# fy-vision/DiGA

Measured on AMD Instinct MI355X. Metric: 768x768 19-class crops/sec (DiGA warm-up step), higher is better.
Workload: dtype f32; 1 GPU; configs[1]: ResNet-101 DeepLabV2 DiGA warm-up (student + EMA teacher, KL distill), synthetic GTA5-shape 768x768, batch 8 per GPU; global_batch=8, parallelism=dp1

## Files before the change

### diga_amd/csrc/conv.hip

```cpp
#include <stdlib.h>
#include <string.h>

#include <algorithm>
#include <atomic>

#include "common.h"

namespace diga {

using f32x16 = __attribute__((ext_vector_type(16))) float;
using f32x4nt = __attribute__((ext_vector_type(4))) float;

__device__ __forceinline__ void store4_stream(float* p, float x, float y, float z, float w) {
#if defined(DIGA_PROBE_NOSTORE)
    if (x == 1.2345e38f) *p = y + z + w;
#elif defined(DIGA_PROBE_PLAINSTORE)
    *reinterpret_cast<float4*>(p) = make_float4(x, y, z, w);
#else
    __builtin_nontemporal_store((f32x4nt){x, y, z, w}, reinterpret_cast<f32x4nt*>(p));
#endif
}

constexpr int kBK = 32;

// ... 1051 lines not shown
#pragma unroll
        for (int j = 0; j < NT; ++j)
#pragma unroll
            for (int e = 0; e < 4; ++e)
                stage[((wm & 1) * 64 + i * 16 + (lane >> 4) * 4 + e) * LDS_LD + wn * 32 * TN + j * 16 + (lane & 15)] = acc[i][j][e];
    __syncthreads();
    drain_stage<2, TN, EPI>(stage, a, m0 + h * 128, n0, t, tile_m * 2 + h, m0 + h * 128 < a.M);
}

#if defined(DIGA_PROBE_STAMP)
__device__ unsigned long long g_probe_stamps[8192 * 6];
#define DIGA_STAMP(slot_)                                                                                                  \
    do {                                                                                                                   \
        if (wv == 0 && lane == 0 && blockIdx.x < 8192) {                                                                   \
            __builtin_amdgcn_sched_barrier(0);                                                                             \
            g_probe_stamps[blockIdx.x * 6 + (slot_)] = __builtin_amdgcn_s_memrealtime();                                   \
            __builtin_amdgcn_sched_barrier(0);                                                                             \
        }                                                                                                                  \
    } while (0)
#else
#define DIGA_STAMP(slot_) do { } while (0)
#endif

#ifndef DIGA_FWD_DMA_MINW
#define DIGA_FWD_DMA_MINW 3
#endif
template <bool EPI = false>
__global__ __launch_bounds__(768, DIGA_FWD_DMA_MINW) void conv_fwd_dma_kernel(ConvArgs a) {
    constexpr int BM = 256, BN = 128;
    constexpr int A_BYTES = BM * 128, B_BYTES = BN * 128, STAGE = A_BYTES + B_BYTES;
    extern __shared__ __align__(16) unsigned char smem_b[];
    const int lane = threadIdx.x & 63, wv = threadIdx.x >> 6;
    const bool loader = wv >= 8;
    DIGA_STAMP(0);
    const int wg = xcd_remap(blockIdx.x, gridDim.x);
    const int tile_n = wg % a.tiles_n, tile_m = wg / a.tiles_n;
    const int m0 = tile_m * BM, n0 = tile_n * BN;
    const int RS = a.R * a.S;
    const int cchunks = a.Cin / 32;
    const uint64_t live = RS <= 64 ? live_taps(a, m0, BM) : ~0ull;
    const int ntaps = RS <= 64 ? __builtin_popcountll(live) : RS;
    const int ksteps = ntaps * cchunks;

    if (loader) {
        const int lw = wv - 8;
        const unsigned char* in_b = reinterpret_cast<const unsigned char*>(a.in);
        const int lrow = lane >> 3;
        int pixbase[8], yx0[8];
        bool mok[8];
        const int HoWo = a.Ho * a.Wo;
#pragma unroll
        for (int j = 0; j < 8; ++j) {
            const int m = m0 + lw * 64 + 8 * j + lrow;
            mok[j] = m < a.M;
            const int mm = mok[j] ? m : a.M - 1;
            const int img = mm / HoWo, rem = mm - img * HoWo;
            const int ho = rem / a.Wo, wo = rem - ho * a.Wo;
            pixbase[j] = img * a.Hi * a.Wi;
            yx0[j] = ((ho * a.sy + a.oy0) << 16) | ((wo * a.sx + a.ox0) & 0xffff);
        }
        const int64_t rowb = (int64_t)a.in_ld * 4;
        const unsigned char* pa[8];
        const unsigned char* pb[4];
#pragma unroll
        for (int c = 0; c < 4; ++c) {
            const int r = lw * 32 + 8 * c + lrow, co = n0 + r;
            const int chunk = (lane & 7) ^ ((r >> 1) & 7);
            const float* wbase = a.wb_tiles > 0 ? a.wgt + (int64_t)(tile_m / a.wb_tiles) * a.wb_stride : a.wgt;
            pb[c] = co < a.Cout ? reinterpret_cast<const unsigned char*>(wbase) + (int64_t)co * RS * a.Cin * 4 + chunk * 16 : nullptr;
        }
        uint64_t todo = live;
        int l_tap = 0, l_cc = 0;
        auto next_tap = [&]() {
            if (RS <= 64) {
                l_tap = __builtin_ctzll(todo);
                todo &= todo - 1;
            } else {
                ++l_tap;
            }
        };
        auto set_tap = [&](int tap) {
            const int r = tap / a.S, q = tap - r * a.S;
            const int dy = r * a.ody, dx = q * a.odx;
#pragma unroll
            for (int j = 0; j < 8; ++j) {
                const int iy = (yx0[j] >> 16) + dy, ix = (int)(short)(yx0[j] & 0xffff) + dx;
                int cy, cx;
                const bool ok = map_tap(a, iy, ix, cy, cx) && mok[j];
                const int chunk = (lane & 7) ^ (((8 * j + lrow) >> 1) & 7);
                pa[j] = ok ? in_b + (int64_t)(pixbase[j] + cy * a.Wi + cx) * rowb + chunk * 16 : nullptr;
            }
        };
        int issued = 0;
        auto issue = [&](int buf) {
            unsigned char* stage = smem_b + buf * STAGE;
#pragma unroll
            for (int j = 0; j < 8; ++j) {
                const unsigned char* src = pa[j] != nullptr ? pa[j] + l_cc * 128 : g_zero16;
                __builtin_amdgcn_global_load_lds((const __attribute__((address_space(1))) void*)src,
                                                 (__attribute__((address_space(3))) void*)(stage + (lw * 64 + 8 * j) * 128), 16, 0, 0);
            }
            const int64_t boff = ((int64_t)l_tap * a.Cin + l_cc * 32) * 4;
#pragma unroll
            for (int c = 0; c < 4; ++c) {
                const unsigned char* src = pb[c] != nullptr ? pb[c] + boff : g_zero16;
                __builtin_amdgcn_global_load_lds((const __attribute__((address_space(1))) void*)src,
                                                 (__attribute__((address_space(3))) void*)(stage + A_BYTES + (lw * 32 + 8 * c) * 128), 16, 0, 0);
            }
            ++issued;
            if (++l_cc == cchunks) {
                l_cc = 0;
                if (issued < ksteps) {
                    next_tap();
                    set_tap(l_tap);
                }
            }
        };
        auto wait_next = [&](bool newest_in_flight) {
            if (newest_in_flight) asm volatile("s_waitcnt vmcnt(12)" ::: "memory");
            else asm volatile("s_waitcnt vmcnt(0)" ::: "memory");
            __builtin_amdgcn_s_barrier();
        };
        if (RS <= 64) next_tap();
        set_tap(l_tap);
        issue(0);
        if (ksteps > 1) issue(1);
        wait_next(ksteps > 1);
        int nx = 2;
        for (int ks = 0; ks < ksteps; ++ks) {
            const bool ahead = ks + 2 < ksteps;
            if (ahead) issue(nx);
            wait_next(ahead);
            nx = nx == 2 ? 0 : nx + 1;
        }
        return;
    }

    const int wm = wv >> 1, wn = wv & 1;
    f32x16 acc[2][2];
#pragma unroll
    for (int i = 0; i < 2; ++i)
#pragma unroll
        for (int j = 0; j < 2; ++j)
// ... 737 lines not shown
#pragma unroll
            for (int j = 0; j < NT; ++j) acc[i][j] = __builtin_amdgcn_mfma_f32_16x16x32_bf16(ah, bh[j], acc[i][j], 0, 0, 0);
        }
        asm volatile("s_waitcnt lgkmcnt(0)" ::: "memory");
        __builtin_amdgcn_s_barrier();
        cur = cur == 2 ? 0 : cur + 1;
    }

    float* out = a.slab + (int64_t)split * a.Cout * RS * a.Cin;
#pragma unroll
    for (int j = 0; j < NT; ++j) {
        const int c = c0 + wn * 64 + j * 16 + (lane & 15);
#pragma unroll
        for (int i = 0; i < MT; ++i) {
#pragma unroll
            for (int e = 0; e < 4; ++e) {
                const int kk = k0 + wm * 128 + i * 16 + (lane >> 4) * 4 + e;
                if (kk < a.Cout && c < a.Cin) out[((int64_t)kk * RS + tap) * a.Cin + c] = acc[i][j][e];
            }
        }
    }
}

__global__ __launch_bounds__(768, 3) void conv_wgrad_dma_kernel(WgradArgs a) {
    constexpr int BM = 256, BN = 128;
    constexpr int A_ROW = BM * 4, B_ROW = BN * 4;
    constexpr int A_BYTES = kBK * A_ROW, B_BYTES = kBK * B_ROW, STAGE = A_BYTES + B_BYTES;
    extern __shared__ __align__(16) unsigned char smem_b[];
    const int lane = threadIdx.x & 63, wv = threadIdx.x >> 6;
    const bool loader = wv >= 8;
    const int RS = a.R * a.S;
    int wg = xcd_remap(blockIdx.x, gridDim.x);
    const int tile_n = wg % a.tiles_n;
    wg /= a.tiles_n;
    const int tile_m = wg % a.tiles_m;
    wg /= a.tiles_m;
    const int tap = wg % RS;
    const int split = wg / RS;
    const int k0 = tile_m * BM, c0 = tile_n * BN;
    const int p_begin = split * a.steps_per_split * kBK;
    int p_end = p_begin + a.steps_per_split * kBK;
    if (p_end > a.M) p_end = a.M;
    const int ksteps = p_end > p_begin ? (p_end - p_begin + kBK - 1) / kBK : 0;

    if (loader) {
        const int lw = wv - 8;
        const unsigned char* dyb = reinterpret_cast<const unsigned char*>(a.dy) + ((int64_t)k0 + tap * a.dy_tap_stride) * 4;
        const unsigned char* xb = reinterpret_cast<const unsigned char*>(a.x) + ((int64_t)c0 + tap * a.x_tap_stride) * 4;
        const int64_t dy_rowb = (int64_t)a.dy_ld * 4, x_rowb = (int64_t)a.x_ld * 4;
        const int* tab = a.ptab != nullptr ? a.ptab + (int64_t)tap * a.M_pad : nullptr;
        const int b_half = lane >> 5;
        const int b_src = (((lane & 31) ^ (b_half << 3)) << 4);
        int bidx[4];
        auto load_idx = [&](int ks) {
#pragma unroll
            for (int j = 0; j < 4; ++j) {
                const int p = p_begin + ks * kBK + 8 * lw + 2 * j + b_half;
                bidx[j] = p < p_end ? (tab != nullptr ? tab[p] : p) : -1;
            }
        };
        auto issue = [&](int ks, int stg) {
            unsigned char* stage = smem_b + stg * STAGE;
#pragma unroll
            for (int j = 0; j < 8; ++j) {
                const int row = 8 * lw + j;
                const int p = min(p_begin + ks * kBK + row, a.M - 1);
                const unsigned char* src = dyb + p * dy_rowb + ((lane ^ ((j & 1) << 3)) << 4);
                __builtin_amdgcn_global_load_lds((const __attribute__((address_space(1))) void*)src,
                                                 (__attribute__((address_space(3))) void*)(stage + row * A_ROW), 16, 0, 0);
            }
#pragma unroll
            for (int j = 0; j < 4; ++j) {
                const unsigned char* src = bidx[j] >= 0 ? xb + bidx[j] * x_rowb + b_src : g_zero16;
                __builtin_amdgcn_global_load_lds((const __attribute__((address_space(1))) void*)src,
                                                 (__attribute__((address_space(3))) void*)(stage + A_BYTES + (8 * lw + 2 * j) * B_ROW), 16, 0, 0);
            }
        };
        auto wait_next = [&](bool newest_in_flight) {
            if (newest_in_flight) asm volatile("s_waitcnt vmcnt(12)" ::: "memory");
            else asm volatile("s_waitcnt vmcnt(0)" ::: "memory");
            __builtin_amdgcn_s_barrier();
        };
        if (ksteps > 0) {
            load_idx(0);
            issue(0, 0);
            if (ksteps > 1) {
                load_idx(1);
                issue(1, 1);
            }
        }
        wait_next(ksteps > 1);
        int nx = 2;
        for (int ks = 0; ks < ksteps; ++ks) {
            const bool ahead = ks + 2 < ksteps;
            if (ahead) {
                load_idx(ks + 2);
                issue(ks + 2, nx);
            }
            wait_next(ahead);
            nx = nx == 2 ? 0 : nx + 1;
        }
        return;
    }
// ... 131 lines not shown
    DIGA_REQUIRE(!e->mask_bits || e->mask_bits_ld * 8 >= a.Cout, DIGA_EINVAL, "%s: bad mask_bits", who);
    DIGA_REQUIRE(!e->relu_ab || (e->x && aligned16(e->relu_ab)), DIGA_EINVAL, "%s: relu_ab needs x", who);
    DIGA_REQUIRE(!e->partials || (e->x && e->mean && e->invstd && aligned16(e->mean) && aligned16(e->invstd)), DIGA_EINVAL,
                 "%s: partials need x, mean and invstd", who);
    a.e_add = e->addend; a.e_add_ld = (int)e->addend_ld;
    a.e_masky = e->mask_y; a.e_masky_ld = (int)e->mask_ld;
    a.e_maskbits = e->mask_bits; a.e_maskbits_ld = (int)e->mask_bits_ld;
    a.e_x = e->x; a.e_x_ld = (int)e->x_ld;
    a.e_relu_ab = e->relu_ab; a.e_mean = e->mean; a.e_invstd = e->invstd; a.e_partials = e->partials;
    return DIGA_OK;
}

struct GemmArgs {
    const float* A;
    const float* W;
    float* out;
    int M, K, Cout, tiles_m, tiles_n, wb_tiles;
    int64_t wb_stride;
    int64_t a_ld, out_ld;
    const float* bias;
    float* stats;
};

__global__ __launch_bounds__(768, 3) void gemm_f32_persistent_kernel(GemmArgs g) {
    constexpr int A_BYTES = 256 * 128, B_BYTES = 128 * 128, STAGE = A_BYTES + B_BYTES;
    extern __shared__ __align__(16) unsigned char smem_b[];
    const int lane = threadIdx.x & 63, wv = threadIdx.x >> 6;
    const bool loader = wv >= 8;
    const int total = g.tiles_m * g.tiles_n;
    const int xcd = blockIdx.x & 7, slot = blockIdx.x >> 3, nslots = gridDim.x >> 3;
    const int q = total >> 3, r = total & 7;
    const int start = xcd < r ? xcd * (q + 1) : r * (q + 1) + (xcd - r) * q, len = q + (xcd < r ? 1 : 0);
    const int nmine = slot < len ? (len - slot + nslots - 1) / nslots : 0;
    if (nmine == 0) return;
    const int ksteps = g.K / 32;
    const int total_steps = nmine * ksteps;
    const int64_t rowb = g.a_ld * 4, wrowb = (int64_t)g.K * 4;

    if (loader) {
        const int lw = wv - 8;
        const int lrow = lane >> 3;
        const unsigned char* pa[8];
        const unsigned char* pb[4];
        int l_it = 0, l_cc = 0, issued = 0;
        auto set_tile = [&](int it) {
            const int t = start + slot + nslots * it;
            const int tile_n = t % g.tiles_n, tile_m = t / g.tiles_n;
            const int row0 = tile_m * 256 + lw * 64 + lrow;
            const unsigned char* ab = reinterpret_cast<const unsigned char*>(g.A) + (int64_t)row0 * rowb;
            const unsigned char* wb = reinterpret_cast<const unsigned char*>(g.W + (g.wb_tiles > 0 ? (int64_t)(tile_m / g.wb_tiles) * g.wb_stride : 0)) +
                                      (int64_t)(tile_n * 128 + lw * 32 + lrow) * wrowb;
#pragma unroll
            for (int j = 0; j < 8; ++j)
                pa[j] = row0 + 8 * j < g.M ? ab + (int64_t)(8 * j) * rowb + (((lane & 7) ^ (((8 * j + lrow) >> 1) & 7)) << 4) : nullptr;
#pragma unroll
            for (int c = 0; c < 4; ++c) pb[c] = wb + (int64_t)(8 * c) * wrowb + (((lane & 7) ^ (((8 * c + lrow) >> 1) & 7)) << 4);
        };
        auto issue = [&](int buf) {
            unsigned char* stage = smem_b + buf * STAGE;
#pragma unroll
            for (int j = 0; j < 8; ++j) {
                const unsigned char* src = pa[j] != nullptr ? pa[j] + l_cc * 128 : g_zero16;
                __builtin_amdgcn_global_load_lds((const __attribute__((address_space(1))) void*)src,
                                                 (__attribute__((address_space(3))) void*)(stage + (lw * 64 + 8 * j) * 128), 16, 0, 0);
            }
#pragma unroll
            for (int c = 0; c < 4; ++c)
                __builtin_amdgcn_global_load_lds((const __attribute__((address_space(1))) void*)(pb[c] + l_cc * 128),
                                                 (__attribute__((address_space(3))) void*)(stage + A_BYTES + (lw * 32 + 8 * c) * 128), 16, 0, 0);
            ++issued;
            if (++l_cc == ksteps) {
                l_cc = 0;
                if (++l_it < nmine) set_tile(l_it);
            }
        };
        auto wait_next = [&](bool newest_in_flight) {
            if (newest_in_flight) asm volatile("s_waitcnt vmcnt(12)" ::: "memory");
            else asm volatile("s_waitcnt vmcnt(0)" ::: "memory");
            __builtin_amdgcn_s_barrier();
        };
        set_tile(0);
        issue(0);
        if (total_steps > 1) issue(1);
        wait_next(total_steps > 1);
        int nx = 2;
        for (int gs = 0; gs < total_steps; ++gs) {
            const bool ahead = gs + 2 < total_steps;
            if (ahead) issue(nx);
            wait_next(ahead);
            nx = nx == 2 ? 0 : nx + 1;
        }
        return;
    }

    const int wm = wv >> 1, wn = wv & 1;
    f32x16 acc[2][2];
#pragma unroll
    for (int i = 0; i < 2; ++i)
#pragma unroll
        for (int j = 0; j < 2; ++j)
#pragma unroll
// ... 106 lines not shown
                 "gemm_batched_f32_dma: rows %% 256, K %% 32, Cout %% 4 required");
    const int64_t M = rows_per_batch * batches;
    DIGA_REQUIRE(M / 256 < 32768 && M < (1ll << 31), DIGA_EINVAL, "gemm_batched_f32_dma: too many rows");
    ConvArgs a;
    a.in = A; a.wgt = W; a.wgt_hi = nullptr; a.wgt_lo = nullptr; a.wgt_img = nullptr; a.bias = nullptr; a.out = out; a.stats = nullptr;
    a.N = 1; a.Hi = (int)(M / 256); a.Wi = 256; a.Cin = (int)K; a.in_ld = (int)K;
    a.Ho = a.Hi; a.Wo = 256; a.Cout = (int)Cout; a.out_ld = (int)Cout;
    a.R = 1; a.S = 1; a.sy = 1; a.sx = 1; a.oy0 = 0; a.ox0 = 0; a.ody = 1; a.odx = 1;
    a.M = (int)M; a.tiles_m = (int)ceil_div(M, 128); a.tiles_n = (int)ceil_div(Cout, 128); a.all_inside = 1;
    a.pad_reflect = 0; a.up_shift = 0; a.act = 0;
    a.e_add = a.e_masky = a.e_x = a.e_relu_ab = a.e_mean = a.e_invstd = nullptr;
    a.e_partials = nullptr; a.e_maskbits = nullptr;
    a.e_add_ld = a.e_masky_ld = a.e_x_ld = a.e_maskbits_ld = 0;
    a.wb_tiles = (int)(rows_per_batch / 256);
    a.wb_stride = Cout * K;
    const unsigned grid = (unsigned)((M / 256) * a.tiles_n);
    const size_t sh = 3 * (256 + 128) * 128;
    if (Cout % 128 == 0 && grid >= 512 && M * Cout < (1ll << 32)) {
        GemmArgs g;
        g.A = A; g.W = W; g.out = out; g.M = (int)M; g.K = (int)K; g.Cout = (int)Cout;
        g.tiles_m = (int)(M / 256); g.tiles_n = a.tiles_n; g.wb_tiles = a.wb_tiles; g.wb_stride = a.wb_stride;
        g.a_ld = K; g.out_ld = Cout; g.bias = nullptr; g.stats = nullptr;
        (void)hipFuncSetAttribute((const void*)gemm_f32_persistent_kernel, hipFuncAttributeMaxDynamicSharedMemorySize, (int)sh);
        hipLaunchKernelGGL(gemm_f32_persistent_kernel, dim3(256), dim3(768), sh, st, g);
        return DIGA_OK;
    }
    (void)hipFuncSetAttribute((const void*)conv_fwd_dma_kernel<false>, hipFuncAttributeMaxDynamicSharedMemorySize, (int)sh);
    hipLaunchKernelGGL(conv_fwd_dma_kernel<false>, dim3(grid), dim3(768), sh, st, a);
    return DIGA_OK;
}

bool pointwise_persistent_ok(int64_t M, int64_t Hi, int64_t Wi, int64_t Cin, int64_t Ho, int64_t Wo, int64_t Cout, int64_t R,
                             int64_t S, int64_t sy, int64_t sx, int64_t oy0, int64_t ox0) {
    return R == 1 && S == 1 && sy == 1 && sx == 1 && oy0 == 0 && ox0 == 0 && Hi == Ho && Wi == Wo && Cin % 32 == 0 &&
           Cout % 128 == 0 && ceil_div(M, 256) * (Cout / 128) >= 512;
}

}

using namespace diga;

static int conv2d_f32_impl(const float* in, const float* wgt, const float* bias, float* out, int64_t N,
                                    int64_t Hi, int64_t Wi, int64_t Cin, int64_t in_ld, int64_t Ho, int64_t Wo,
                                    int64_t Cout, int64_t out_ld, int64_t R, int64_t S, int64_t stride_y,
                                    int64_t stride_x, int64_t off_y0, int64_t off_x0, int64_t off_dy, int64_t off_dx,
                                    float* stats_partial, int prof_tag, void* stream, const diga_bwd_epilogue_t* epi,
                                    const diga_conv_options_t* opts = nullptr) {
    DIGA_REQUIRE(in && wgt && out, DIGA_EINVAL, "conv2d: null pointer");
    DIGA_REQUIRE(N > 0 && Hi > 0 && Wi > 0 && Ho > 0 && Wo > 0 && Cout > 0 && R > 0 && S > 0, DIGA_EINVAL, "conv2d: bad shape");
    int rc = check_conv_common("conv2d", Cin, in_ld, out_ld, Cout, in, wgt, out);
    if (rc) return rc;
// ... 16 lines not shown
    ProfScope prof(prof_tag == DIGA_PROF_CONV_BWD_DATA ? DIGA_PROF_CONV_BWD_DATA : DIGA_PROF_CONV_FWD, st,
                   2.0 * (double)a.M * (double)Cout * (double)(R * S) * (double)Cin);
#define DIGA_LAUNCH_K(KERNEL_, THREADS_, SH_)                                                                          \
    do {                                                                                                               \
        (void)hipFuncSetAttribute((const void*)KERNEL_, hipFuncAttributeMaxDynamicSharedMemorySize, (int)(SH_));        \
        hipLaunchKernelGGL(KERNEL_, dim3((unsigned)(a.tiles_m * a.tiles_n)), dim3(THREADS_), (SH_), st, a);             \
    } while (0)
#define DIGA_FWD_LAUNCH(TN_, BK_)                                                                                      \
    do {                                                                                                               \
        const size_t sh = (size_t)(2 * 128 * (BK_ + 4) + 2 * 64 * TN_ * (BK_ + 4)) * sizeof(float);                     \
        if (epi != nullptr) DIGA_LAUNCH_K((conv_fwd_kernel<TN_, 32, true>), 256, sh);                                   \
        else DIGA_LAUNCH_K((conv_fwd_kernel<TN_, BK_, false>), 256, sh);                                                \
    } while (0)
    if (pointwise_persistent_ok(N * Ho * Wo, Hi, Wi, Cin, Ho, Wo, Cout, R, S, stride_y, stride_x, off_y0, off_x0) &&
        epi == nullptr && !(opts && (opts->reflect_pad || opts->upsample_shift || opts->activation))) {
        DIGA_REQUIRE((int64_t)a.M * out_ld < (1ll << 32), DIGA_EINVAL, "conv2d_nhwc_f32: output beyond 2^32 elements (the pointwise kernel "
                     "addresses it with 32-bit element offsets)");
        GemmArgs g;
        g.A = in; g.W = wgt; g.out = out; g.M = a.M; g.K = (int)Cin; g.Cout = (int)Cout;
        g.tiles_m = (int)ceil_div(a.M, 256); g.tiles_n = (int)(Cout / 128); g.wb_tiles = 0; g.wb_stride = 0;
        g.a_ld = in_ld; g.out_ld = out_ld; g.bias = bias; g.stats = stats_partial;
        const size_t shp = 3 * (256 + 128) * 128;
        (void)hipFuncSetAttribute((const void*)gemm_f32_persistent_kernel, hipFuncAttributeMaxDynamicSharedMemorySize, (int)shp);
        hipLaunchKernelGGL(gemm_f32_persistent_kernel, dim3(256), dim3(768), shp, st, g);
        return launch_status("diga_conv2d_nhwc_f32");
    }
    if (a.M >= 256 && Cout >= 256 && R * S * Cin >= 256) {
        a.tiles_n = (int)ceil_div(Cout, 128);
        const unsigned grid = (unsigned)(ceil_div(a.M, 256) * a.tiles_n);
        const size_t sh = 3 * (256 + 128) * 128;
        if (epi != nullptr) {
            (void)hipFuncSetAttribute((const void*)conv_fwd_dma_kernel<true>, hipFuncAttributeMaxDynamicSharedMemorySize, (int)sh);
            hipLaunchKernelGGL(conv_fwd_dma_kernel<true>, dim3(grid), dim3(768), sh, st, a);
        } else {
            (void)hipFuncSetAttribute((const void*)conv_fwd_dma_kernel<false>, hipFuncAttributeMaxDynamicSharedMemorySize, (int)sh);
            hipLaunchKernelGGL(conv_fwd_dma_kernel<false>, dim3(grid), dim3(768), sh, st, a);
        }
    } else if (Cout > 64) {
        a.tiles_n = (int)ceil_div(Cout, 128);
        DIGA_FWD_LAUNCH(2, 32);
    } else {
        a.tiles_n = 1;
        DIGA_FWD_LAUNCH(1, 32);
    }
#undef DIGA_FWD_LAUNCH
    return launch_status("diga_conv2d_nhwc_f32");
}


extern "C" int diga_conv2d_nhwc_f32(const float* in, const float* wgt, const float* bias, float* out, int64_t N,
                                    int64_t Hi, int64_t Wi, int64_t Cin, int64_t in_ld, int64_t Ho, int64_t Wo,
                                    int64_t Cout, int64_t out_ld, int64_t R, int64_t S, int64_t stride_y,
                                    int64_t stride_x, int64_t off_y0, int64_t off_x0, int64_t off_dy, int64_t off_dx,
                                    float* stats_partial, int prof_tag, void* stream) {
    return conv2d_f32_impl(in, wgt, bias, out, N, Hi, Wi, Cin, in_ld, Ho, Wo, Cout, out_ld, R, S, stride_y, stride_x, off_y0, off_x0,
                           off_dy, off_dx, stats_partial, prof_tag, stream, nullptr);
}

extern "C" int diga_conv2d_nhwc_f32_epi(const float* in, const float* wgt, float* out, int64_t N, int64_t Hi, int64_t Wi,
// ... 303 lines not shown
}

namespace diga {
size_t wgrad_batched_slab_bytes(int64_t rows, int batches, int64_t Cout, int64_t Cin) {
    return wgrad_slab_bytes(plan_wgrad_wide(rows, Cout, Cin, batches), Cout, Cin, batches);
}
int wgrad_batched_f32_dma(const float* Z, const float* V, float* dU, float* slab, int64_t rows, int batches, int64_t Cout,
                          int64_t Cin, hipStream_t st) {
    DIGA_REQUIRE(rows > 0 && rows % 32 == 0 && Cout % 256 == 0 && Cin % 128 == 0 && batches > 0 && rows < (1ll << 31), DIGA_EINVAL,
                 "wgrad_batched_f32_dma: rows %% 32, Cout %% 256, Cin %% 128 required");
    const WgradPlan p = plan_wgrad_wide(rows, Cout, Cin, batches);
    WgradArgs a;
    a.dy = Z; a.x = V; a.slab = p.splits > 1 ? slab : dU;
    a.N = 1; a.Hi = 1; a.Wi = (int)rows; a.Cin = (int)Cin; a.x_ld = (int)Cin;
    a.Ho = 1; a.Wo = (int)rows; a.Cout = (int)Cout; a.dy_ld = (int)Cout;
    a.R = 1; a.S = batches; a.sy = 1; a.sx = 1; a.oy0 = 0; a.ox0 = 0; a.ody = 1; a.odx = 1;
    a.M = (int)rows; a.tiles_m = p.tiles_m; a.tiles_n = p.tiles_n; a.splits = p.splits; a.steps_per_split = p.steps_per_split;
    a.ptab = nullptr; a.zeros = nullptr; a.M_pad = (int)rows;
    a.dy_tap_stride = rows * Cout;
    a.x_tap_stride = rows * Cin;
    const unsigned grid = (unsigned)((int64_t)p.tiles_m * p.tiles_n * batches * p.splits);
    const size_t shd = (size_t)3 * kBK * (256 + 128) * 4;
    (void)hipFuncSetAttribute((const void*)conv_wgrad_dma_kernel, hipFuncAttributeMaxDynamicSharedMemorySize, (int)shd);
    hipLaunchKernelGGL(conv_wgrad_dma_kernel, dim3(grid), dim3(768), shd, st, a);
    if (p.splits > 1) {
        const int64_t n4 = Cout * batches * Cin / 4;
        hipLaunchKernelGGL(slab_reduce_kernel, dim3((unsigned)ceil_div(n4, 256)), dim3(256), 0, st, (const float*)slab, dU, n4, p.splits);
    }
    return DIGA_OK;
}

}

extern "C" size_t diga_conv2d_wgrad_workspace_bytes(int64_t N, int64_t Ho, int64_t Wo, int64_t Cout, int64_t Cin,
                                                    int64_t R, int64_t S) {
    const int64_t M = N * Ho * Wo, RS = R * S;
    const size_t s0 = wgrad_slab_bytes(plan_wgrad(M, Cout, Cin, RS, false), Cout, Cin, RS);
    size_t s1 = wgrad_slab_bytes(plan_wgrad(M, Cout, Cin, RS, true), Cout, Cin, RS);
    if (wgrad_dma_ok(M, Cout, Cin)) s1 = std::max(s1, wgrad_slab_bytes(plan_wgrad_wide(M, Cout, Cin, RS), Cout, Cin, RS));
    return (s0 > s1 ? s0 : s1) + (size_t)RS * wgrad_mpad(M) * sizeof(int) + 64;
}

extern "C" int diga_conv2d_wgrad_nhwc_f32(const float* dy, const float* x, float* dw, void* workspace,
                                          size_t workspace_bytes, int64_t N, int64_t Hi, int64_t Wi, int64_t Cin,
                                          int64_t x_ld, int64_t Ho, int64_t Wo, int64_t Cout, int64_t dy_ld, int64_t R,
                                          int64_t S, int64_t stride_y, int64_t stride_x, int64_t off_y0,
                                          int64_t off_x0, int64_t off_dy, int64_t off_dx, int math, void* stream) {
// ... 37 lines not shown
        a.ptab = tab;
        a.zeros = zeros;
        const size_t shw = (size_t)2 * (256 + 64 * p.tn) * kRowB;
        if (p.tn == 2) {
            (void)hipFuncSetAttribute((const void*)conv_wgrad_x3w_kernel<2>, hipFuncAttributeMaxDynamicSharedMemorySize, (int)shw);
            hipLaunchKernelGGL((conv_wgrad_x3w_kernel<2>), dim3(grid), dim3(256), shw, st, a);
        } else {
            (void)hipFuncSetAttribute((const void*)conv_wgrad_x3w_kernel<1>, hipFuncAttributeMaxDynamicSharedMemorySize, (int)shw);
            hipLaunchKernelGGL((conv_wgrad_x3w_kernel<1>), dim3(grid), dim3(256), shw, st, a);
        }
    } else
    {
    if (f32_tab) {
        int* tab = reinterpret_cast<int*>(static_cast<char*>(workspace) + slab_bytes);
        float* zeros = reinterpret_cast<float*>(tab + RS * M_pad);
        hipLaunchKernelGGL(wgrad_pixtab_kernel, dim3((unsigned)ceil_div(M_pad, 256), (unsigned)RS), dim3(256), 0, st, tab, zeros,
                           (int)M, (int)M_pad, (int)Ho, (int)Wo, (int)Hi, (int)Wi, (int)S, (int)stride_y, (int)stride_x,
                           (int)off_y0, (int)off_x0, (int)off_dy, (int)off_dx);
        a.ptab = tab;
    }
    if (dma) {
        const size_t shd = (size_t)3 * kBK * (256 + 128) * 4;
        (void)hipFuncSetAttribute((const void*)conv_wgrad_dma_kernel, hipFuncAttributeMaxDynamicSharedMemorySize, (int)shd);
        hipLaunchKernelGGL(conv_wgrad_dma_kernel, dim3(grid), dim3(768), shd, st, a);
    } else {
    const size_t sh = (size_t)(4 * kBK * kLDW) * sizeof(float);
#define DIGA_WGRAD_LAUNCH(TM_, TN_)                                                                                   \
    do {                                                                                                               \
        (void)hipFuncSetAttribute((const void*)conv_wgrad_kernel<TM_, TN_>, hipFuncAttributeMaxDynamicSharedMemorySize, (int)sh); \
        hipLaunchKernelGGL((conv_wgrad_kernel<TM_, TN_>), dim3(grid), dim3(256), sh, st, a);                            \
    } while (0)
#define DIGA_WGRAD_X3_LAUNCH(TM_, TN_)                                                                                \
    do {                                                                                                               \
        const size_t shx = (size_t)2 * (2 * 64 * TM_ * kRowB + 2 * 64 * TN_ * kRowB);                                   \
        (void)hipFuncSetAttribute((const void*)conv_wgrad_x3_kernel<TM_, TN_>, hipFuncAttributeMaxDynamicSharedMemorySize, (int)shx); \
        hipLaunchKernelGGL((conv_wgrad_x3_kernel<TM_, TN_>), dim3(grid), dim3(256), shx, st, a);                        \
    } while (0)
    if (x3) {
        if (p.tm == 2 && p.tn == 2) DIGA_WGRAD_X3_LAUNCH(2, 2);
        else if (p.tm == 2) DIGA_WGRAD_X3_LAUNCH(2, 1);
        else if (p.tn == 2) DIGA_WGRAD_X3_LAUNCH(1, 2);
        else DIGA_WGRAD_X3_LAUNCH(1, 1);
    } else {
        if (p.tm == 2 && p.tn == 2) DIGA_WGRAD_LAUNCH(2, 2);
        else if (p.tm == 2) DIGA_WGRAD_LAUNCH(2, 1);
        else if (p.tn == 2) DIGA_WGRAD_LAUNCH(1, 2);
        else DIGA_WGRAD_LAUNCH(1, 1);
// ... 130 lines not shown
```

### diga_amd/csrc/winograd.hip

```cpp
#include "common.h"

namespace diga {

int gemm_batched_f32_dma(const float* A, int64_t rows_per_batch, int batches, int64_t K, const float* W, int64_t Cout,
                         float* out, hipStream_t st);
size_t wgrad_batched_slab_bytes(int64_t rows, int batches, int64_t Cout, int64_t Cin);
int wgrad_batched_f32_dma(const float* Z, const float* V, float* dU, float* slab, int64_t rows, int batches, int64_t Cout,
                          int64_t Cin, hipStream_t st);

namespace wino {

struct WinoGeom {
    int N, H, W, d;
    int m;
    int tys, txs;
    int64_t T, Tp;
};

int phase_tiles(int len, int d, int m) {
    int s = 0;
    for (int a = 0; a < d; ++a) {
        const int n = len > a ? (len - a + d - 1) / d : 0;
        s += (n + m - 1) / m;
    }
// ... 463 lines not shown
                y = y >= H ? 2 * (H - 1) - y : y;
            }
            const bool ok = xok && (reflect || (unsigned)y < (unsigned)H);
            const int yc = min(max(y, 0), H - 1);
            const V v = *reinterpret_cast<const V*>(x + ((int64_t)(img * H + yc) * W + xc) * ld + c);
            p[i] = ok ? v : z;
        }
        V col[A];
        Xf<M>::bt(p, col);
#pragma unroll
        for (int i = 0; i < A; ++i) m[i][j] = col[i];
    }
    float* o = Vo + t * C + c;
    const int64_t plane = Tp * C;
#pragma unroll
    for (int i = 0; i < A; ++i) {
        V row[A];
        Xf<M>::bt(m[i], row);
#pragma unroll
        for (int j = 0; j < A; ++j) wino_in_store<V>(o + (A * i + j) * plane, row[j]);
    }
}

template <int M, typename V>
__device__ __forceinline__ void winoM_load_rows(const float* __restrict__ src, int64_t plane, V (*s)[M + 2]) {
    constexpr int A = M + 2;
    const float* p[A];
#pragma unroll
    for (int i = 0; i < A; ++i) p[i] = src + (int64_t)(A * i) * plane;
#pragma unroll
    for (int j = 0; j < A; ++j) {
        V m[A];
#pragma unroll
        for (int i = 0; i < A; ++i) {
            m[i] = nt_loadv<V>(p[i]);
            p[i] += plane;
        }
        V col[M];
        Xf<M>::at(m, col);
#pragma unroll
        for (int i = 0; i < M; ++i) s[i][j] = col[i];
    }
}

template <int M, typename V>
__global__ __launch_bounds__(256) void winoM_output_kernel(const float* __restrict__ Mb, const int4* __restrict__ tab,
// ... 247 lines not shown
        V u[A];
#pragma unroll
        for (int i = 0; i < A; ++i) u[i] = *reinterpret_cast<const V*>(src + (int64_t)(A * i + j) * Cin);
        V col[3];
        Xf<M>::gt(u, col);
#pragma unroll
        for (int r = 0; r < 3; ++r) t[r][j] = col[r];
    }
    float* o = dw + (int64_t)co * 9 * Cin + c;
#pragma unroll
    for (int r = 0; r < 3; ++r) {
        V row[3];
        Xf<M>::gt(t[r], row);
#pragma unroll
        for (int q = 0; q < 3; ++q) *reinterpret_cast<V*>(o + (int64_t)(3 * r + q) * Cin) = row[q];
    }
}

template <int M>
static void launch_input_m(const float* x, int64_t ld, const int4* tab, float* V, int64_t Tp, int64_t C, int64_t H, int64_t W, int64_t d,
                           hipStream_t st, int reflect) {
    using VT = typename Vec<M>::In;
    constexpr int VW = sizeof(VT) / 4;
    const dim3 grid((unsigned)ceil_div(Tp * (C / VW), 256));
    if (reflect)
        hipLaunchKernelGGL((winoM_input_kernel<M, VT, true>), grid, dim3(256), 0, st, x, ld, tab, V, Tp, (int)C, (int)H, (int)W, (int)d);
    else
        hipLaunchKernelGGL((winoM_input_kernel<M, VT, false>), grid, dim3(256), 0, st, x, ld, tab, V, Tp, (int)C, (int)H, (int)W, (int)d);
}
static void launch_input(int64_t tile, const float* x, int64_t ld, const int4* tab, float* V, int64_t Tp, int64_t C, int64_t H, int64_t W,
                         int64_t d, hipStream_t st, int reflect = 0) {
    if (tile == 6) launch_input_m<6>(x, ld, tab, V, Tp, C, H, W, d, st, reflect);
    else if (tile == 4) launch_input_m<4>(x, ld, tab, V, Tp, C, H, W, d, st, reflect);
    else
        hipLaunchKernelGGL(wino_input_kernel, dim3((unsigned)ceil_div(Tp * (C / 4), 256)), dim3(256), 0, st, x, ld, tab, V, Tp, (int)C,
                           (int)H, (int)W, (int)d);
}
template <int M>
static void launch_weight_m(const float* w, float* U, int64_t Cout, int64_t Cin, int flip, hipStream_t st) {
    hipLaunchKernelGGL(winoM_weight_kernel<M>, dim3((unsigned)ceil_div(Cout * (Cin / 4), 256)), dim3(256), 0, st, w, U, (int)Cout, (int)Cin, flip);
}
template <int M>
static void launch_output_m(const float* Mb, const int4* tab, const float* bias, float* out, int64_t out_ld, const WinoGeom& g, int64_t Cout,
                            hipStream_t st) {
    using VT = typename Vec<M>::Out;
    constexpr int VW = sizeof(VT) / 4;
// ... 43 lines not shown
        hipLaunchKernelGGL((winoM_output_epi2_kernel<M, VT, TL, ADD, MASK, true>), grid, dim3(256), 0, st, Mb, tab, out, out_ld, g.T, g.Tp,
                           (int)Cout, g.H, g.W, g.d, tpb, ep);
    else
        hipLaunchKernelGGL((winoM_output_epi2_kernel<M, VT, TL, ADD, MASK, false>), grid, dim3(256), 0, st, Mb, tab, out, out_ld, g.T, g.Tp,
                           (int)Cout, g.H, g.W, g.d, tpb, ep);
}
template <int M, bool ADD>
static void launch_output_epi2_mask(const float* Mb, const int4* tab, float* out, int64_t out_ld, const WinoGeom& g, int64_t Cout, int64_t G,
                                    int tpb, const WinoEpi& ep, hipStream_t st) {
    if (ep.masky != nullptr) launch_output_epi2_sums<M, ADD, 1>(Mb, tab, out, out_ld, g, Cout, G, tpb, ep, st);
    else if (ep.maskbits != nullptr) launch_output_epi2_sums<M, ADD, 2>(Mb, tab, out, out_ld, g, Cout, G, tpb, ep, st);
    else if (ep.relu_ab != nullptr) launch_output_epi2_sums<M, ADD, 3>(Mb, tab, out, out_ld, g, Cout, G, tpb, ep, st);
    else launch_output_epi2_sums<M, ADD, 0>(Mb, tab, out, out_ld, g, Cout, G, tpb, ep, st);
}
template <int M>
static void launch_output_epi2_m(const float* Mb, const int4* tab, float* out, int64_t out_ld, const WinoGeom& g, int64_t Cout, int64_t G,
                                 int tpb, const WinoEpi& ep, hipStream_t st) {
    if (ep.add != nullptr) launch_output_epi2_mask<M, true>(Mb, tab, out, out_ld, g, Cout, G, tpb, ep, st);
    else launch_output_epi2_mask<M, false>(Mb, tab, out, out_ld, g, Cout, G, tpb, ep, st);
}

template <int M>
static void launch_dy_m(const float* dy, int64_t dy_ld, const int4* tab, float* Z, const WinoGeom& g, int64_t Cout, hipStream_t st) {
    using VT = typename Vec<M>::Dy;
    constexpr int VW = sizeof(VT) / 4;
    hipLaunchKernelGGL((winoM_dy_kernel<M, VT>), dim3((unsigned)ceil_div(g.Tp * (Cout / VW), 256)), dim3(256), 0, st, dy, dy_ld, tab, Z, g.Tp,
                       (int)Cout, g.H, g.W, g.d);
}
template <int M>
static void launch_dw_m(const float* dU, float* dw, int64_t Cout, int64_t Cin, hipStream_t st) {
    hipLaunchKernelGGL((winoM_dw_kernel<M, float2>), dim3((unsigned)ceil_div(Cout * (Cin / 2), 256)), dim3(256), 0, st, dU, dw, (int)Cout, (int)Cin);
}

struct WinoWgradLayout {
    size_t tab, V, Z, dU, slab, total;
};
WinoWgradLayout wino_wgrad_layout(const WinoGeom& g, int64_t Cin, int64_t Cout, bool with_v) {
    WinoWgradLayout l;
    size_t o = 0;
    l.tab = o; o += (size_t)g.Tp * sizeof(int4);
    l.V = o; o += with_v ? (size_t)products(g.m) * g.Tp * Cin * sizeof(float) : 0;
    l.Z = o; o += (size_t)products(g.m) * g.Tp * Cout * sizeof(float);
    l.dU = o; o += (size_t)products(g.m) * Cout * Cin * sizeof(float);
    l.slab = o; o += wgrad_batched_slab_bytes(g.Tp, products(g.m), Cout, Cin);
    l.total = o + 64;
    return l;
}

struct WinoLayout {
    size_t tab, U, V, M, total;
// ... 223 lines not shown
```

Baseline: 19.78 crops/s.

## Halve DMA loader waves in conv/GEMM kernels and add split Winograd F6 transforms

```diff
diff --git a/diga_amd/csrc/conv.hip b/diga_amd/csrc/conv.hip
--- a/diga_amd/csrc/conv.hip
+++ b/diga_amd/csrc/conv.hip
@@ -1097,12 +1097,31 @@
 #define DIGA_STAMP(slot_) do { } while (0)
 #endif
 
+#ifndef DIGA_FWD_DMA_LOADERS
+#define DIGA_FWD_DMA_LOADERS 2
+#endif
+#ifndef DIGA_WGRAD_DMA_LOADERS
+#define DIGA_WGRAD_DMA_LOADERS 2
+#endif
+#ifndef DIGA_GEMM_LOADERS
+#define DIGA_GEMM_LOADERS 2
+#endif
+constexpr int kFwdDmaLoaders = DIGA_FWD_DMA_LOADERS, kWgradDmaLoaders = DIGA_WGRAD_DMA_LOADERS, kGemmPersistentLoaders = DIGA_GEMM_LOADERS;
+static_assert((kFwdDmaLoaders == 2 || kFwdDmaLoaders == 4) && (kWgradDmaLoaders == 2 || kWgradDmaLoaders == 4) &&
+                  (kGemmPersistentLoaders == 2 || kGemmPersistentLoaders == 4),
+              "two or four loader waves: 48 loads per stage of one wave would need a different wait count scheme (vmcnt holds 63)");
+template <int N>
+__device__ __forceinline__ void dma_wait_vmcnt() {
+    asm volatile("s_waitcnt vmcnt(%0)" ::"n"(N) : "memory");
+}
+
 #ifndef DIGA_FWD_DMA_MINW
 #define DIGA_FWD_DMA_MINW 3
 #endif
 template <bool EPI = false>
-__global__ __launch_bounds__(768, DIGA_FWD_DMA_MINW) void conv_fwd_dma_kernel(ConvArgs a) {
+__global__ __launch_bounds__(512 + 64 * kFwdDmaLoaders, DIGA_FWD_DMA_MINW) void conv_fwd_dma_kernel(ConvArgs a) {
     constexpr int BM = 256, BN = 128;
+    constexpr int NL = kFwdDmaLoaders, LA = BM / 8 / NL, LB = BN / 8 / NL;
     constexpr int A_BYTES = BM * 128, B_BYTES = BN * 128, STAGE = A_BYTES + B_BYTES;
     extern __shared__ __align__(16) unsigned char smem_b[];
     const int lane = threadIdx.x & 63, wv = threadIdx.x >> 6;
@@ -1121,32 +1140,27 @@
         const int lw = wv - 8;
         const unsigned char* in_b = reinterpret_cast<const unsigned char*>(a.in);
         const int lrow = lane >> 3;
-        int pixbase[8], yx0[8];
-        bool mok[8];
+        int pixbase[LA], yx0[LA];
         const int HoWo = a.Ho * a.Wo;
 #pragma unroll
-        for (int j = 0; j < 8; ++j) {
-            const int m = m0 + lw * 64 + 8 * j + lrow;
-            mok[j] = m < a.M;
-            const int mm = mok[j] ? m : a.M - 1;
+        for (int j = 0; j < LA; ++j) {
+            const int m = m0 + 8 * (lw * LA + j) + lrow;
+            const bool mok = m < a.M;
+            const int mm = mok ? m : a.M - 1;
             const int img = mm / HoWo, rem = mm - img * HoWo;
             const int ho = rem / a.Wo, wo = rem - ho * a.Wo;
-            pixbase[j] = img * a.Hi * a.Wi;
+            pixbase[j] = mok ? img * a.Hi * a.Wi : -1;
             yx0[j] = ((ho * a.sy + a.oy0) << 16) | ((wo * a.sx + a.ox0) & 0xffff);
         }
         const int64_t rowb = (int64_t)a.in_ld * 4;
-        const unsigned char* pa[8];
-        const unsigned char* pb[4];
-#pragma unroll
-        for (int c = 0; c < 4; ++c) {
-            const int r = lw * 32 + 8 * c + lrow, co = n0 + r;
-            const int chunk = (lane & 7) ^ ((r >> 1) & 7);
-            const float* wbase = a.wb_tiles > 0 ? a.wgt + (int64_t)(tile_m / a.wb_tiles) * a.wb_stride : a.wgt;
-            pb[c] = co < a.Cout ? reinterpret_cast<const unsigned char*>(wbase) + (int64_t)co * RS * a.Cin * 4 + chunk * 16 : nullptr;
-        }
+        const unsigned char* pa[LA];
+        const int brow0 = 8 * lw * LB + lrow;
+        const int64_t wrow8 = (int64_t)8 * RS * a.Cin * 4;
+        const unsigned char* pb0 = reinterpret_cast<const unsigned char*>(a.wb_tiles > 0 ? a.wgt + (int64_t)(tile_m / a.wb_tiles) * a.wb_stride : a.wgt) +
+                                   (int64_t)(n0 + brow0) * RS * a.Cin * 4;
         uint64_t todo = live;
         int l_tap = 0, l_cc = 0;
-        auto next_tap = [&]() {
+        auto next_tap = [&]() __attribute__((always_inline)) {
             if (RS <= 64) {
                 l_tap = __builtin_ctzll(todo);
                 todo &= todo - 1;
@@ -1154,33 +1168,34 @@
                 ++l_tap;
             }
         };
-        auto set_tap = [&](int tap) {
+        auto set_tap = [&](int tap) __attribute__((always_inline)) {
             const int r = tap / a.S, q = tap - r * a.S;
             const int dy = r * a.ody, dx = q * a.odx;
 #pragma unroll
-            for (int j = 0; j < 8; ++j) {
+            for (int j = 0; j < LA; ++j) {
                 const int iy = (yx0[j] >> 16) + dy, ix = (int)(short)(yx0[j] & 0xffff) + dx;
                 int cy, cx;
-                const bool ok = map_tap(a, iy, ix, cy, cx) && mok[j];
+                const bool ok = map_tap(a, iy, ix, cy, cx) && pixbase[j] >= 0;
                 const int chunk = (lane & 7) ^ (((8 * j + lrow) >> 1) & 7);
                 pa[j] = ok ? in_b + (int64_t)(pixbase[j] + cy * a.Wi + cx) * rowb + chunk * 16 : nullptr;
             }
         };
         int issued = 0;
-        auto issue = [&](int buf) {
+        auto issue = [&](int buf) __attribute__((always_inline)) {
             unsigned char* stage = smem_b + buf * STAGE;
 #pragma unroll
-            for (int j = 0; j < 8; ++j) {
+            for (int j = 0; j < LA; ++j) {
                 const unsigned char* src = pa[j] != nullptr ? pa[j] + l_cc * 128 : g_zero16;
                 __builtin_amdgcn_global_load_lds((const __attribute__((address_space(1))) void*)src,
-                                                 (__attribute__((address_space(3))) void*)(stage + (lw * 64 + 8 * j) * 128), 16, 0, 0);
+                                                 (__attribute__((address_space(3))) void*)(stage + 8 * (lw * LA + j) * 128), 16, 0, 0);
             }
             const int64_t boff = ((int64_t)l_tap * a.Cin + l_cc * 32) * 4;
 #pragma unroll
-            for (int c = 0; c < 4; ++c) {
-                const unsigned char* src = pb[c] != nullptr ? pb[c] + boff : g_zero16;
+            for (int c = 0; c < LB; ++c) {
+                const int chunk = (lane & 7) ^ (((8 * c + lrow) >> 1) & 7);
+                const unsigned char* src = n0 + brow0 + 8 * c < a.Cout ? pb0 + c * wrow8 + chunk * 16 + boff : g_zero16;
                 __builtin_amdgcn_global_load_lds((const __attribute__((address_space(1))) void*)src,
-                                                 (__attribute__((address_space(3))) void*)(stage + A_BYTES + (lw * 32 + 8 * c) * 128), 16, 0, 0);
+                                                 (__attribute__((address_space(3))) void*)(stage + A_BYTES + 8 * (lw * LB + c) * 128), 16, 0, 0);
             }
             ++issued;
             if (++l_cc == cchunks) {
@@ -1191,9 +1206,9 @@
                 }
             }
         };
-        auto wait_next = [&](bool newest_in_flight) {
-            if (newest_in_flight) asm volatile("s_waitcnt vmcnt(12)" ::: "memory");
-            else asm volatile("s_waitcnt vmcnt(0)" ::: "memory");
+        auto wait_next = [&](bool newest_in_flight) __attribute__((always_inline)) {
+            if (newest_in_flight) dma_wait_vmcnt<LA + LB>();
+            else dma_wait_vmcnt<0>();
             __builtin_amdgcn_s_barrier();
         };
         if (RS <= 64) next_tap();
@@ -1977,8 +1992,9 @@
     }
 }
 
-__global__ __launch_bounds__(768, 3) void conv_wgrad_dma_kernel(WgradArgs a) {
+__global__ __launch_bounds__(512 + 64 * kWgradDmaLoaders, 3) void conv_wgrad_dma_kernel(WgradArgs a) {
     constexpr int BM = 256, BN = 128;
+    constexpr int NL = kWgradDmaLoaders, RPL = kBK / NL;
     constexpr int A_ROW = BM * 4, B_ROW = BN * 4;
     constexpr int A_BYTES = kBK * A_ROW, B_BYTES = kBK * B_ROW, STAGE = A_BYTES + B_BYTES;
     extern __shared__ __align__(16) unsigned char smem_b[];
@@ -2004,36 +2020,37 @@
         const unsigned char* xb = reinterpret_cast<const unsigned char*>(a.x) + ((int64_t)c0 + tap * a.x_tap_stride) * 4;
         const int64_t dy_rowb = (int64_t)a.dy_ld * 4, x_rowb = (int64_t)a.x_ld * 4;
         const int* tab = a.ptab != nullptr ? a.ptab + (int64_t)tap * a.M_pad : nullptr;
+        static_assert(kBK == 32 && RPL % 2 == 0, "conv_wgrad_dma_kernel: 32-pixel K-steps, an even number of rows per loader wave");
         const int b_half = lane >> 5;
         const int b_src = (((lane & 31) ^ (b_half << 3)) << 4);
-        int bidx[4];
+        int bidx[RPL / 2];
         auto load_idx = [&](int ks) {
 #pragma unroll
-            for (int j = 0; j < 4; ++j) {
-                const int p = p_begin + ks * kBK + 8 * lw + 2 * j + b_half;
+            for (int j = 0; j < RPL / 2; ++j) {
+                const int p = p_begin + ks * kBK + RPL * lw + 2 * j + b_half;
                 bidx[j] = p < p_end ? (tab != nullptr ? tab[p] : p) : -1;
             }
         };
         auto issue = [&](int ks, int stg) {
             unsigned char* stage = smem_b + stg * STAGE;
 #pragma unroll
-            for (int j = 0; j < 8; ++j) {
-                const int row = 8 * lw + j;
+            for (int j = 0; j < RPL; ++j) {
+                const int row = RPL * lw + j;
                 const int p = min(p_begin + ks * kBK + row, a.M - 1);
                 const unsigned char* src = dyb + p * dy_rowb + ((lane ^ ((j & 1) << 3)) << 4);
                 __builtin_amdgcn_global_load_lds((const __attribute__((address_space(1))) void*)src,
                                                  (__attribute__((address_space(3))) void*)(stage + row * A_ROW), 16, 0, 0);
             }
 #pragma unroll
-            for (int j = 0; j < 4; ++j) {
+            for (int j = 0; j < RPL / 2; ++j) {
                 const unsigned char* src = bidx[j] >= 0 ? xb + bidx[j] * x_rowb + b_src : g_zero16;
                 __builtin_amdgcn_global_load_lds((const __attribute__((address_space(1))) void*)src,
-                                                 (__attribute__((address_space(3))) void*)(stage + A_BYTES + (8 * lw + 2 * j) * B_ROW), 16, 0, 0);
+                                                 (__attribute__((address_space(3))) void*)(stage + A_BYTES + (RPL * lw + 2 * j) * B_ROW), 16, 0, 0);
             }
         };
         auto wait_next = [&](bool newest_in_flight) {
-            if (newest_in_flight) asm volatile("s_waitcnt vmcnt(12)" ::: "memory");
-            else asm volatile("s_waitcnt vmcnt(0)" ::: "memory");
+            if (newest_in_flight) dma_wait_vmcnt<RPL + RPL / 2>();
+            else dma_wait_vmcnt<0>();
             __builtin_amdgcn_s_barrier();
         };
         if (ksteps > 0) {
@@ -2211,8 +2228,9 @@
     float* stats;
 };
 
-__global__ __launch_bounds__(768, 3) void gemm_f32_persistent_kernel(GemmArgs g) {
+__global__ __launch_bounds__(512 + 64 * kGemmPersistentLoaders, 3) void gemm_f32_persistent_kernel(GemmArgs g) {
     constexpr int A_BYTES = 256 * 128, B_BYTES = 128 * 128, STAGE = A_BYTES + B_BYTES;
+    constexpr int NL = kGemmPersistentLoaders, LA = 256 / 8 / NL, LB = 128 / 8 / NL;
     extern __shared__ __align__(16) unsigned char smem_b[];
     const int lane = threadIdx.x & 63, wv = threadIdx.x >> 6;
     const bool loader = wv >= 8;
@@ -2229,34 +2247,34 @@
     if (loader) {
         const int lw = wv - 8;
         const int lrow = lane >> 3;
-        const unsigned char* pa[8];
-        const unsigned char* pb[4];
+        const unsigned char* pa[LA];
+        const unsigned char* pb[LB];
         int l_it = 0, l_cc = 0, issued = 0;
         auto set_tile = [&](int it) {
             const int t = start + slot + nslots * it;
             const int tile_n = t % g.tiles_n, tile_m = t / g.tiles_n;
-            const int row0 = tile_m * 256 + lw * 64 + lrow;
+            const int row0 = tile_m * 256 + lw * (8 * LA) + lrow;
             const unsigned char* ab = reinterpret_cast<const unsigned char*>(g.A) + (int64_t)row0 * rowb;
             const unsigned char* wb = reinterpret_cast<const unsigned char*>(g.W + (g.wb_tiles > 0 ? (int64_t)(tile_m / g.wb_tiles) * g.wb_stride : 0)) +
-                                      (int64_t)(tile_n * 128 + lw * 32 + lrow) * wrowb;
-#pragma unroll
-            for (int j = 0; j < 8; ++j)
+                                      (int64_t)(tile_n * 128 + lw * (8 * LB) + lrow) * wrowb;
+#pragma unroll
+            for (int j = 0; j < LA; ++j)
                 pa[j] = row0 + 8 * j < g.M ? ab + (int64_t)(8 * j) * rowb + (((lane & 7) ^ (((8 * j + lrow) >> 1) & 7)) << 4) : nullptr;
 #pragma unroll
-            for (int c = 0; c < 4; ++c) pb[c] = wb + (int64_t)(8 * c) * wrowb + (((lane & 7) ^ (((8 * c + lrow) >> 1) & 7)) << 4);
+            for (int c = 0; c < LB; ++c) pb[c] = wb + (int64_t)(8 * c) * wrowb + (((lane & 7) ^ (((8 * c + lrow) >> 1) & 7)) << 4);
         };
         auto issue = [&](int buf) {
             unsigned char* stage = smem_b + buf * STAGE;
 #pragma unroll
-            for (int j = 0; j < 8; ++j) {
+            for (int j = 0; j < LA; ++j) {
                 const unsigned char* src = pa[j] != nullptr ? pa[j] + l_cc * 128 : g_zero16;
                 __builtin_amdgcn_global_load_lds((const __attribute__((address_space(1))) void*)src,
-                                                 (__attribute__((address_space(3))) void*)(stage + (lw * 64 + 8 * j) * 128), 16, 0, 0);
-            }
-#pragma unroll
-            for (int c = 0; c < 4; ++c)
+                                                 (__attribute__((address_space(3))) void*)(stage + 8 * (lw * LA + j) * 128), 16, 0, 0);
+            }
+#pragma unroll
+            for (int c = 0; c < LB; ++c)
                 __builtin_amdgcn_global_load_lds((const __attribute__((address_space(1))) void*)(pb[c] + l_cc * 128),
-                                                 (__attribute__((address_space(3))) void*)(stage + A_BYTES + (lw * 32 + 8 * c) * 128), 16, 0, 0);
+                                                 (__attribute__((address_space(3))) void*)(stage + A_BYTES + 8 * (lw * LB + c) * 128), 16, 0, 0);
             ++issued;
             if (++l_cc == ksteps) {
                 l_cc = 0;
@@ -2264,8 +2282,8 @@
             }
         };
         auto wait_next = [&](bool newest_in_flight) {
-            if (newest_in_flight) asm volatile("s_waitcnt vmcnt(12)" ::: "memory");
-            else asm volatile("s_waitcnt vmcnt(0)" ::: "memory");
+            if (newest_in_flight) dma_wait_vmcnt<LA + LB>();
+            else dma_wait_vmcnt<0>();
             __builtin_amdgcn_s_barrier();
         };
         set_tile(0);
@@ -2418,11 +2436,11 @@
         g.tiles_m = (int)(M / 256); g.tiles_n = a.tiles_n; g.wb_tiles = a.wb_tiles; g.wb_stride = a.wb_stride;
         g.a_ld = K; g.out_ld = Cout; g.bias = nullptr; g.stats = nullptr;
         (void)hipFuncSetAttribute((const void*)gemm_f32_persistent_kernel, hipFuncAttributeMaxDynamicSharedMemorySize, (int)sh);
-        hipLaunchKernelGGL(gemm_f32_persistent_kernel, dim3(256), dim3(768), sh, st, g);
+        hipLaunchKernelGGL(gemm_f32_persistent_kernel, dim3(256), dim3(512 + 64 * kGemmPersistentLoaders), sh, st, g);
         return DIGA_OK;
     }
     (void)hipFuncSetAttribute((const void*)conv_fwd_dma_kernel<false>, hipFuncAttributeMaxDynamicSharedMemorySize, (int)sh);
-    hipLaunchKernelGGL(conv_fwd_dma_kernel<false>, dim3(grid), dim3(768), sh, st, a);
+    hipLaunchKernelGGL(conv_fwd_dma_kernel<false>, dim3(grid), dim3(512 + 64 * kFwdDmaLoaders), sh, st, a);
     return DIGA_OK;
 }
 
@@ -2485,7 +2503,7 @@
         g.a_ld = in_ld; g.out_ld = out_ld; g.bias = bias; g.stats = stats_partial;
         const size_t shp = 3 * (256 + 128) * 128;
         (void)hipFuncSetAttribute((const void*)gemm_f32_persistent_kernel, hipFuncAttributeMaxDynamicSharedMemorySize, (int)shp);
-        hipLaunchKernelGGL(gemm_f32_persistent_kernel, dim3(256), dim3(768), shp, st, g);
+        hipLaunchKernelGGL(gemm_f32_persistent_kernel, dim3(256), dim3(512 + 64 * kGemmPersistentLoaders), shp, st, g);
         return launch_status("diga_conv2d_nhwc_f32");
     }
     if (a.M >= 256 && Cout >= 256 && R * S * Cin >= 256) {
@@ -2494,10 +2512,10 @@
         const size_t sh = 3 * (256 + 128) * 128;
         if (epi != nullptr) {
             (void)hipFuncSetAttribute((const void*)conv_fwd_dma_kernel<true>, hipFuncAttributeMaxDynamicSharedMemorySize, (int)sh);
-            hipLaunchKernelGGL(conv_fwd_dma_kernel<true>, dim3(grid), dim3(768), sh, st, a);
+            hipLaunchKernelGGL(conv_fwd_dma_kernel<true>, dim3(grid), dim3(512 + 64 * kFwdDmaLoaders), sh, st, a);
         } else {
             (void)hipFuncSetAttribute((const void*)conv_fwd_dma_kernel<false>, hipFuncAttributeMaxDynamicSharedMemorySize, (int)sh);
-            hipLaunchKernelGGL(conv_fwd_dma_kernel<false>, dim3(grid), dim3(768), sh, st, a);
+            hipLaunchKernelGGL(conv_fwd_dma_kernel<false>, dim3(grid), dim3(512 + 64 * kFwdDmaLoaders), sh, st, a);
         }
     } else if (Cout > 64) {
         a.tiles_n = (int)ceil_div(Cout, 128);
@@ -2847,7 +2865,7 @@
     const unsigned grid = (unsigned)((int64_t)p.tiles_m * p.tiles_n * batches * p.splits);
     const size_t shd = (size_t)3 * kBK * (256 + 128) * 4;
     (void)hipFuncSetAttribute((const void*)conv_wgrad_dma_kernel, hipFuncAttributeMaxDynamicSharedMemorySize, (int)shd);
-    hipLaunchKernelGGL(conv_wgrad_dma_kernel, dim3(grid), dim3(768), shd, st, a);
+    hipLaunchKernelGGL(conv_wgrad_dma_kernel, dim3(grid), dim3(512 + 64 * kWgradDmaLoaders), shd, st, a);
     if (p.splits > 1) {
         const int64_t n4 = Cout * batches * Cin / 4;
         hipLaunchKernelGGL(slab_reduce_kernel, dim3((unsigned)ceil_div(n4, 256)), dim3(256), 0, st, (const float*)slab, dU, n4, p.splits);
@@ -2931,7 +2949,7 @@
     if (dma) {
         const size_t shd = (size_t)3 * kBK * (256 + 128) * 4;
         (void)hipFuncSetAttribute((const void*)conv_wgrad_dma_kernel, hipFuncAttributeMaxDynamicSharedMemorySize, (int)shd);
-        hipLaunchKernelGGL(conv_wgrad_dma_kernel, dim3(grid), dim3(768), shd, st, a);
+        hipLaunchKernelGGL(conv_wgrad_dma_kernel, dim3(grid), dim3(512 + 64 * kWgradDmaLoaders), shd, st, a);
     } else {
     const size_t sh = (size_t)(4 * kBK * kLDW) * sizeof(float);
 #define DIGA_WGRAD_LAUNCH(TM_, TN_)                                                                                   \
diff --git a/diga_amd/csrc/winograd.hip b/diga_amd/csrc/winograd.hip
--- a/diga_amd/csrc/winograd.hip
+++ b/diga_amd/csrc/winograd.hip
@@ -509,6 +509,128 @@
     }
 }
 
+__device__ __forceinline__ void wino_half_swap(float& a, float& b) {
+    const auto r = __builtin_amdgcn_permlane32_swap(__float_as_uint(a), __float_as_uint(b), false, false);
+    a = __uint_as_float(r[0]);
+    b = __uint_as_float(r[1]);
+}
+template <bool REFLECT>
+__global__ __launch_bounds__(256) void wino6_input_split_kernel(const float* __restrict__ x, int64_t ld, const int4* __restrict__ tab,
+                                                                float* __restrict__ Vo, int64_t Tp, int C, int H, int W, int d) {
+    constexpr bool reflect = REFLECT;
+    constexpr int A = 8;
+    const int lane = threadIdx.x & 63, h = lane >> 5;
+    const int wv = __builtin_amdgcn_readfirstlane((int)(threadIdx.x >> 6));
+    const int cgn = C >> 5;
+    const int64_t unit = (int64_t)blockIdx.x * 4 + wv;
+    if (unit >= Tp * cgn) return;
+    const int64_t t = unit / cgn;
+    const int c = (int)(unit - t * cgn) * 32 + (lane & 31);
+    const int4 e = tab[t];
+    const int img = max(e.x, 0);
+    float p[4][A], m[A][4];
+#pragma unroll
+    for (int jj = 0; jj < 4; ++jj) {
+        int xx = e.z + (4 * h + jj - 1) * d;
+        if (reflect) {
+            xx = xx < 0 ? -xx : xx;
+            xx = xx >= W ? 2 * (W - 1) - xx : xx;
+        }
+        const bool xok = e.x >= 0 && (reflect || (unsigned)xx < (unsigned)W);
+        const int xc = min(max(xx, 0), W - 1);
+#pragma unroll
+        for (int i = 0; i < A; ++i) {
+            int y = e.y + (i - 1) * d;
+            if (reflect) {
+                y = y < 0 ? -y : y;
+                y = y >= H ? 2 * (H - 1) - y : y;
+            }
+            const bool ok = xok && (reflect || (unsigned)y < (unsigned)H);
+            const int yc = min(max(y, 0), H - 1);
+            const float v = x[((int64_t)(img * H + yc) * W + xc) * ld + c];
+            p[jj][i] = ok ? v : 0.f;
+        }
+    }
+    __builtin_amdgcn_sched_barrier(0);
+#pragma unroll
+    for (int jj = 0; jj < 4; ++jj) {
+        float col[A];
+        Xf<6>::bt(p[jj], col);
+#pragma unroll
+        for (int i = 0; i < A; ++i) m[i][jj] = col[i];
+    }
+#pragma unroll
+    for (int ii = 0; ii < 4; ++ii)
+#pragma unroll
+        for (int jj = 0; jj < 4; ++jj) wino_half_swap(m[ii][jj], m[4 + ii][jj]);
+    const int64_t plane = Tp * C;
+    float* o = Vo + t * C + c + (int64_t)(A * 4 * h) * plane;
+#pragma unroll
+    for (int ii = 0; ii < 4; ++ii) {
+        float in[A], row[A];
+#pragma unroll
+        for (int jj = 0; jj < 4; ++jj) {
+            in[jj] = m[ii][jj];
+            in[4 + jj] = m[4 + ii][jj];
+        }
+        Xf<6>::bt(in, row);
+#pragma unroll
+        for (int j = 0; j < A; ++j) nt_store4(o + (A * ii + j) * plane, row[j]);
+    }
+}
+
+__global__ __launch_bounds__(256) void wino6_dy_split_kernel(const float* __restrict__ dy, int64_t ld, const int4* __restrict__ tab,
+                                                             float* __restrict__ Z, int64_t Tp, int K, int H, int W, int d) {
+    constexpr int M = 6, A = 8;
+    const int lane = threadIdx.x & 63, h = lane >> 5;
+    const int wv = __builtin_amdgcn_readfirstlane((int)(threadIdx.x >> 6));
+    const int kgn = K >> 5;
+    const int64_t unit = (int64_t)blockIdx.x * 4 + wv;
+    if (unit >= Tp * kgn) return;
+    const int64_t t = unit / kgn;
+    const int k = (int)(unit - t * kgn) * 32 + (lane & 31);
+    const int4 e = tab[t];
+    const int img = max(e.x, 0);
+    float g[3][M], r[A][3];
+#pragma unroll
+    for (int jj = 0; jj < 3; ++jj) {
+        const int xx = e.z + (3 * h + jj) * d, xc = min(xx, W - 1);
+#pragma unroll
+        for (int i = 0; i < M; ++i) {
+            const int yy = e.y + i * d;
+            const bool ok = e.x >= 0 && yy < H && xx < W;
+            const float v = dy[((int64_t)(img * H + min(yy, H - 1)) * W + xc) * ld + k];
+            g[jj][i] = ok ? v : 0.f;
+        }
+    }
+    __builtin_amdgcn_sched_barrier(0);
+#pragma unroll
+    for (int jj = 0; jj < 3; ++jj) {
+        float col[A];
+        Xf<6>::a(g[jj], col);
+#pragma unroll
+        for (int i = 0; i < A; ++i) r[i][jj] = col[i];
+    }
+#pragma unroll
+    for (int ii = 0; ii < 4; ++ii)
+#pragma unroll
+        for (int jj = 0; jj < 3; ++jj) wino_half_swap(r[ii][jj], r[4 + ii][jj]);
+    const int64_t plane = Tp * K;
+    float* o = Z + t * K + k + (int64_t)(A * 4 * h) * plane;
+#pragma unroll
+    for (int ii = 0; ii < 4; ++ii) {
+        float in[M], row[A];
+#pragma unroll
+        for (int jj = 0; jj < 3; ++jj) {
+            in[jj] = r[ii][jj];
+            in[3 + jj] = r[4 + ii][jj];
+        }
+        Xf<6>::a(in, row);
+#pragma unroll
+        for (int j = 0; j < A; ++j) nt_store4(o + (A * ii + j) * plane, row[j]);
+    }
+}
+
 template <int M, typename V>
 __device__ __forceinline__ void winoM_load_rows(const float* __restrict__ src, int64_t plane, V (*s)[M + 2]) {
     constexpr int A = M + 2;
@@ -802,6 +924,16 @@
                            hipStream_t st, int reflect) {
     using VT = typename Vec<M>::In;
     constexpr int VW = sizeof(VT) / 4;
+    if constexpr (M == 6) {
+        if (C % 64 == 0) {
+            const dim3 sgrid((unsigned)ceil_div(Tp * (C / 32), 4));
+            if (reflect)
+                hipLaunchKernelGGL(wino6_input_split_kernel<true>, sgrid, dim3(256), 0, st, x, ld, tab, V, Tp, (int)C, (int)H, (int)W, (int)d);
+            else
+                hipLaunchKernelGGL(wino6_input_split_kernel<false>, sgrid, dim3(256), 0, st, x, ld, tab, V, Tp, (int)C, (int)H, (int)W, (int)d);
+            return;
+        }
+    }
     const dim3 grid((unsigned)ceil_div(Tp * (C / VW), 256));
     if (reflect)
         hipLaunchKernelGGL((winoM_input_kernel<M, VT, true>), grid, dim3(256), 0, st, x, ld, tab, V, Tp, (int)C, (int)H, (int)W, (int)d);
@@ -891,10 +1023,15 @@
 
 template <int M>
 static void launch_dy_m(const float* dy, int64_t dy_ld, const int4* tab, float* Z, const WinoGeom& g, int64_t Cout, hipStream_t st) {
-    using VT = typename Vec<M>::Dy;
-    constexpr int VW = sizeof(VT) / 4;
-    hipLaunchKernelGGL((winoM_dy_kernel<M, VT>), dim3((unsigned)ceil_div(g.Tp * (Cout / VW), 256)), dim3(256), 0, st, dy, dy_ld, tab, Z, g.Tp,
-                       (int)Cout, g.H, g.W, g.d);
+    if constexpr (M == 6) {
+        hipLaunchKernelGGL(wino6_dy_split_kernel, dim3((unsigned)ceil_div(g.Tp * (Cout / 32), 4)), dim3(256), 0, st, dy, dy_ld, tab, Z, g.Tp,
+                           (int)Cout, g.H, g.W, g.d);
+    } else {
+        using VT = typename Vec<M>::Dy;
+        constexpr int VW = sizeof(VT) / 4;
+        hipLaunchKernelGGL((winoM_dy_kernel<M, VT>), dim3((unsigned)ceil_div(g.Tp * (Cout / VW), 256)), dim3(256), 0, st, dy, dy_ld, tab, Z, g.Tp,
+                           (int)Cout, g.H, g.W, g.d);
+    }
 }
 template <int M>
 static void launch_dw_m(const float* dU, float* dw, int64_t Cout, int64_t Cin, hipStream_t st) {
```

After: 19.02 crops/s. 3.8% lower.
